# skywoodsz/qm_control

Hardware: NVIDIA H100
Metric: mpc_wbc_iters_per_s (higher is better)
Workload: dtype f64

## Files before the change

qm_control_b200/csrc/kernels/mpc_kernels.cu:

```cuda
#include <cstdlib>
#include "mpc_api.cuh"
#include "mpc_device.cuh"
#include "node_eval.cuh"
#include "wlinalg.cuh"

namespace qmb {

#ifndef QMB_LQ_WARPS
#define QMB_LQ_WARPS 4
#endif
#ifndef QMB_LQ_MINB
#define QMB_LQ_MINB 4
#endif
constexpr int LQ_WARPS = QMB_LQ_WARPS, LS_WARPS = 4, SETUP_WARPS = 4;
enum { MST_ITER_CAP = 1, MST_OVERFLOW = 2, MST_NAN = 4, MST_NOT_PD = 8, MST_NO_STEP = 16, MST_CONVERGED = 32, MST_NEG_DT = 64 };

__device__ __forceinline__ double interval_start(double t, int ev) { return ev == 2 ? t + WEAK_EPS : t; }
__device__ __forceinline__ double interval_end(double t, int ev) { return ev == 1 ? t - WEAK_EPS : t; }
__device__ __forceinline__ int clamp_events(int ne) { return ne < 0 ? 0 : (ne > EMAX ? EMAX : ne); }
__device__ __forceinline__ int clamp_targets(int nk) { return nk < 1 ? 1 : (nk > KMAX ? KMAX : nk); }
__device__ __forceinline__ int flag_mask(int mode) { int m = 0; for (int i = 0; i < 4; ++i) if (contact_flag(mode, i)) m |= 1 << i; return m; }

struct SetupIdx { int iu, ix; double au, ax; };
__host__ __device__ inline size_t setup_smem_per_warp(int nmax) { return (size_t)nmax * (8 + 8 + 4 + sizeof(SetupIdx) + 4) + 8 * EMAX + 64; }
// ... 59 lines not shown
  ne::NodeRec rec;
  QuadWs quad; LegWs leg[4];
  double x[NX], u[NU];
  double A1r[9 * NX], Ar[9 * NX];
  double Pe_full[NU], rs[NU];
  int dep_idx[MAXDEP], free_idx[MU], col_of_input[NU];
};
static_assert(9 * NX * 8 >= EMAX * 8 + EMAX + 8, "the mode schedule (event times + modes) is staged in the Ar buffer until the flow Jacobians are expanded");
static_assert(sizeof(LqLate) <= 4 * sizeof(ne::FootBlk) && offsetof(ne::NodeRec, foot) == 0, "LqLate overlays the foot blocks of the record");
static_assert(sizeof(LqSmem) % 16 == 0 && offsetof(LqSmem, rec) == 0, "aligned record slice");
static_assert((sizeof(LqSmem) * LQ_WARPS + 1024) * QMB_LQ_MINB <= 232448, "projection kernel: QMB_LQ_MINB CTAs of LQ_WARPS warps per SM (13.8 KB per node: four CTAs of four warps = 16 nodes in flight)");

#ifndef QMB_FL_MINB
#define QMB_FL_MINB 2
#endif
constexpr int FL_WARPS = 4, FL_TILE = 64;
constexpr int FL_SMEM = FL_WARPS * 32 * (FL_TILE + 1) * 8;
__global__ void __launch_bounds__(32 * FL_WARPS, QMB_FL_MINB) mpc_flow_kernel(const DevModel* __restrict__ mdl, int b0, int B, int nmax, MpcProblemDev p, MpcSolutionDev sol, double* __restrict__ rec, const int32_t* __restrict__ status) {
  extern __shared__ __align__(16) unsigned char smem_raw[]; double (*tile)[32][FL_TILE + 1] = reinterpret_cast<double (*)[32][FL_TILE + 1]>(smem_raw);
  const int tid = threadIdx.x, warp = tid >> 5, lane = tid & 31; const long long gid = (long long)blockIdx.x * (32 * FL_WARPS) + tid;
  const int b = b0 + (int)(gid / nmax), k = (int)(gid % nmax);
  const int n = (b < B) ? sol.n_nodes[b] : 0;
  bool work = b < B && k < n && !(status[b] & MST_CONVERGED);
  const bool terminal = work && (k == n - 1);
  if (work && !terminal && sol.event[(size_t)b * nmax + k] == 1) work = false;
  const unsigned active = __ballot_sync(FULL, work); if (!active) return;
  double* row = &tile[warp][lane][0]; double* gbase = rec + ((size_t)b0 * nmax + (size_t)(gid - lane)) * ne::NODE_REC_DBL;
  auto flush = [&](int off, int cnt) {
    __syncwarp();
#pragma unroll 4
    for (int rw = 0; rw < 32; ++rw) if ((active >> rw) & 1u) { double* g = gbase + (size_t)rw * ne::NODE_REC_DBL + off; if (lane < cnt) g[lane] = tile[warp][rw][lane]; if (lane + 32 < cnt) g[lane + 32] = tile[warp][rw][lane + 32]; }
    __syncwarp(); };
  double x[NX], u[NU]; ne::BaseKin bk; ne::FlowAcc acc; double t = 0.0, dt = 0.0;
  if (work) {
    const double* gt = sol.t + (size_t)b * nmax; const int32_t* ge = sol.event + (size_t)b * nmax;
    const double* xk = sol.x + ((size_t)b * nmax + k) * NX; const double* uk = sol.u + ((size_t)b * nmax + k) * NU;
#pragma unroll
    for (int i = 0; i < NX; ++i) { x[i] = xk[i]; u[i] = terminal ? 0.0 : uk[i]; }
    t = interval_start(gt[k], ge[k]); dt = terminal ? 0.0 : interval_end(gt[k + 1], ge[k + 1]) - t;
    ne::base_eval<true>(mdl, x, bk); ne::flow_acc_init(acc);
  }
#pragma unroll 1
  for (int i = 0; i < 4; ++i) {
    if (work) { ne::FootBlk* fb = reinterpret_cast<ne::FootBlk*>(row); double al[9];
      ne::foot_eval<true>(mdl, x, u, bk, i, acc, fb->d, fb->pf, fb->Jl, al, fb->JxF);
      if (!terminal) ne::foot_velocity_1<true>(mdl, x, u, bk, i, fb->d, fb->Jl, al, fb->e, fb->C); }
    flush(i * ne::FOOT_DBL, ne::FOOT_DBL);
  }
  double f1[12];
  if (work) { ne::FlowBlk* fl = reinterpret_cast<ne::FlowBlk*>(row); ne::flow_finish<true>(mdl, x, bk, acc, fl->f, fl);
#pragma unroll
    for (int i = 0; i < 12; ++i) f1[i] = fl->f[i]; }
  flush(4 * ne::FOOT_DBL, ne::FLOW_DBL);
  { ne::EeRec ee;
    if (work) { const int nk = clamp_targets(p.n_target[b]); const ne::TargetSeg sg = ne::target_segment(p.target_times + (size_t)b * KMAX, p.target_states + (size_t)b * KMAX * TARGET_DIM, nk, t);
      double pref[3], qref[4]; ne::target_pose(sg, nk, pref, qref); ne::ee_eval<true>(mdl, x, bk, pref, qref, ee.e, ee.Je);
#pragma unroll
      for (int j = 0; j < 39; ++j) row[j] = reinterpret_cast<const double*>(&ee)[j]; }
    flush(4 * ne::FOOT_DBL + ne::FLOW_DBL, 39);
    if (work) {
#pragma unroll
      for (int j = 0; j < 39; ++j) row[j] = reinterpret_cast<const double*>(&ee)[39 + j]; }
    flush(4 * ne::FOOT_DBL + ne::FLOW_DBL + 39, 39); }
  const bool stage2 = work && !terminal;
  if (stage2) {
    const double cdt = mdl->rk_c * dt;
#pragma unroll
    for (int i = 0; i < NX; ++i) x[i] += cdt * (i < 12 ? f1[i < 12 ? i : 0] : u[i]);
    ne::base_eval<true>(mdl, x, bk); ne::flow_acc_init(acc);
#pragma unroll 1
    for (int i = 0; i < 4; ++i) { ne::Foot2Blk* f2 = reinterpret_cast<ne::Foot2Blk*>(row) + i; ne::foot_eval<true>(mdl, x, u, bk, i, acc, f2->d, nullptr, nullptr, nullptr, f2->JxF); }
  }
  flush(4 * ne::FOOT_DBL + ne::FLOW_DBL + ne::EE_DBL, 4 * ne::FOOT2_DBL);
  if (stage2) { ne::FlowBlk* fl = reinterpret_cast<ne::FlowBlk*>(row); ne::flow_finish<true>(mdl, x, bk, acc, fl->f, fl); }
  flush(4 * ne::FOOT_DBL + ne::FLOW_DBL + ne::EE_DBL + 4 * ne::FOOT2_DBL, ne::FLOW_DBL);
}

__device__ __forceinline__ void expand_flow(const ne::FlowBlk& fb, const double* jxf0, int fstride , double* Ar, int lfp, int lane) {
// ... 544 lines not shown
  }
  armijo = warp_sum(armijo); dxn2 = warp_sum(dxn2); dun2 = warp_sum(dun2);
  __syncthreads();
  if (lane == 0) { sm.red[warp][0] = armijo; sm.red[warp][1] = dxn2; sm.red[warp][2] = dun2; }
  __syncthreads();
  if (tid == 0) { double a = 0, x2 = 0, u2 = 0; for (int w = 0; w < RIC_THREADS / 32; ++w) { a += sm.red[w][0]; x2 += sm.red[w][1]; u2 += sm.red[w][2]; }
    double* rb = robot + (size_t)b * ROBOT_DBL; rb[0] = a; rb[1] = perf[0]; rb[2] = perf[1]; rb[3] = perf[2]; rb[4] = sqrt(x2); rb[5] = sqrt(u2); if (st) atomicOr(&status[b], st); }
}

__device__ __forceinline__ void fixup_inputs(MpcSolutionDev sol, int b, int nmax, int n, int tid, int nthreads) {
  const int32_t* ge = sol.event + (size_t)b * nmax; double* gu = sol.u + (size_t)b * nmax * NU;
  for (int i = tid; i < NU; i += nthreads) for (int k = 1; k < n; ++k) if ((k == n - 1) || (ge[k] == 1)) gu[(size_t)k * NU + i] = gu[(size_t)(k - 1) * NU + i];
}

#ifndef QMB_LS_MINB
#define QMB_LS_MINB 4
#endif
__global__ void __launch_bounds__(32 * LS_WARPS, QMB_LS_MINB) mpc_linesearch_kernel(const DevModel* __restrict__ mdl, int b0, int B, int nmax, MpcProblemDev p, MpcSolutionDev sol, const double* __restrict__ dxo, const double* __restrict__ duo,
                                                                     const double* __restrict__ robot, int32_t* __restrict__ status, double* __restrict__ step_info, int iteration) {
  __shared__ double red[LS_WARPS][3]; __shared__ int decision; __shared__ double s_ev[EMAX]; __shared__ unsigned char s_modes[EMAX + 8];
  const int tid = threadIdx.x, warp = tid >> 5, lane = tid & 31; const int b = b0 + blockIdx.x; if (b >= B) return;
  if (status[b] & MST_CONVERGED) return;
  const int n = sol.n_nodes[b]; const int N = n - 1;
  const double* gt = sol.t + (size_t)b * nmax; const int32_t* ge = sol.event + (size_t)b * nmax;
  double* gx = sol.x + (size_t)b * nmax * NX; double* gu = sol.u + (size_t)b * nmax * NU; const double* gdx = dxo + (size_t)b * nmax * NX; const double* gdu = duo + (size_t)b * nmax * NU;
  const int ne = clamp_events(p.n_events[b]); const double* ev = s_ev; const unsigned char* modes = s_modes;
  if (tid < 32) { const double* gev = p.event_times + (size_t)b * EMAX; const int32_t* gmodes = p.modes + (size_t)b * (EMAX + 1); s_ev[lane] = (lane < ne) ? gev[lane] : 0.0; s_modes[lane] = (unsigned char)((lane <= ne) ? gmodes[lane] : 15); if (lane == 0) s_modes[EMAX] = (unsigned char)((EMAX <= ne) ? gmodes[EMAX] : 15); }
  __syncthreads();
  const int nk = clamp_targets(p.n_target[b]); const double* tt = p.target_times + (size_t)b * KMAX; const double* ts = p.target_states + (size_t)b * KMAX * TARGET_DIM;
  const double* rb = robot + (size_t)b * ROBOT_DBL; const double armijo = rb[0], base_cost = rb[1], base_viol = sqrt(rb[2] + rb[3]), dxn = rb[4], dun = rb[5];
  const bool failed = (status[b] & MST_NOT_PD) != 0;
  double alpha = 1.0; bool accepted = false; double sc = base_cost, sd = rb[2], se = rb[3];
  const double w1 = mdl->rk_w1, w2 = mdl->rk_w2;
  while (!failed) {
    double cost = 0.0, dyn = 0.0, eq = 0.0;
    for (int k = tid; k <= N; k += 32 * LS_WARPS) {
      double xa[NX], ua[NU]; const bool terminal = (k == N);
#pragma unroll
      for (int i = 0; i < NX; ++i) { xa[i] = gx[(size_t)k * NX + i] + alpha * gdx[(size_t)k * NX + i]; ua[i] = terminal ? 0.0 : gu[(size_t)k * NU + i] + alpha * gdu[(size_t)k * NU + i]; }
      if (k == 0) { double s = 0.0; for (int i = 0; i < NX; ++i) { const double d = p.x0[(size_t)b * NX + i] - xa[i]; s = fma(d, d, s); } dyn += s; }
      if (!terminal && ge[k] == 1) { double s = 0.0; for (int i = 0; i < NX; ++i) { const double d = xa[i] - (gx[(size_t)(k + 1) * NX + i] + alpha * gdx[(size_t)(k + 1) * NX + i]); s = fma(d, d, s); } dyn += s; continue; }
      const double t = interval_start(gt[k], ge[k]);
      const double dt = terminal ? 1.0 : interval_end(gt[k + 1], ge[k + 1]) - t; const int mode = mode_at_time(ev, modes, ne, t); const int fm = terminal ? 0 : flag_mask(mode);
      ne::BaseKin bk; ne::FlowAcc acc; double f1[12];
      ne::base_eval<false>(mdl, xa, bk); ne::flow_acc_init(acc);
      { double fe[4][3], pf[4][3];
#pragma unroll 1
        for (int i = 0; i < 4; ++i) { double d[3], Jl[9]; ne::foot_eval<false>(mdl, xa, ua, bk, i, acc, d, pf[i], Jl, nullptr, nullptr); if (!terminal) ne::foot_velocity_1<false>(mdl, xa, ua, bk, i, d, Jl, nullptr, fe[i], nullptr); }
        if (!terminal) eq += dt * ne::equality_ss(mdl, ua, fe, pf, fm, ev, modes, ne, t, nullptr); }
      ne::flow_finish<false>(mdl, xa, bk, acc, f1, nullptr);
      { const ne::TargetSeg sg = ne::target_segment(tt, ts, nk, t); double pref[3], qref[4], ee[6]; ne::target_pose(sg, nk, pref, qref); ne::ee_eval<false>(mdl, xa, bk, pref, qref, ee, nullptr);
        cost += dt * ne::cost_value(mdl, xa, ua, sg, ee, fm, terminal); }
      if (terminal) continue;
      const double cdt = mdl->rk_c * dt;
#pragma unroll
      for (int i = 0; i < NX; ++i) xa[i] += cdt * (i < 12 ? f1[i < 12 ? i : 0] : ua[i]);
      double f2[12]; ne::base_eval<false>(mdl, xa, bk); ne::flow_acc_init(acc);
#pragma unroll 1
      for (int i = 0; i < 4; ++i) { double d[3]; ne::foot_eval<false>(mdl, xa, ua, bk, i, acc, d, nullptr, nullptr, nullptr, nullptr); }
      ne::flow_finish<false>(mdl, xa, bk, acc, f2, nullptr);
      double s = 0.0;
#pragma unroll
      for (int i = 0; i < NX; ++i) { const double fa = (i < 12) ? f1[i < 12 ? i : 0] : ua[i], fb = (i < 12) ? f2[i < 12 ? i : 0] : ua[i];
        const double x0i = gx[(size_t)k * NX + i] + alpha * gdx[(size_t)k * NX + i];
        const double d = x0i + dt * (w1 * fa + w2 * fb) - (gx[(size_t)(k + 1) * NX + i] + alpha * gdx[(size_t)(k + 1) * NX + i]); s = fma(d, d, s); }
      dyn += dt * s;
    }
    cost = warp_sum(cost); dyn = warp_sum(dyn); eq = warp_sum(eq);
    if (lane == 0) { red[warp][0] = cost; red[warp][1] = dyn; red[warp][2] = eq; }
    __syncthreads();
    if (threadIdx.x == 0) {
      double c = 0, dd = 0, e = 0; for (int w = 0; w < LS_WARPS; ++w) { c += red[w][0]; dd += red[w][1]; e += red[w][2]; }
      const double sv = sqrt(dd + e), am = alpha * armijo; bool acc;
      if (sv > mdl->g_max) acc = sv < (1.0 - mdl->gamma_c) * base_viol;
      else if (sv < mdl->g_min && base_viol < mdl->g_min && am < 0.0) acc = c < base_cost + mdl->armijo_factor * am;
      else acc = (c < base_cost - mdl->gamma_c * base_viol) || (sv < (1.0 - mdl->gamma_c) * base_viol);
      red[0][0] = c; red[0][1] = dd; red[0][2] = e;
      int dec = 0; if (acc) dec = 1; else { const double an = alpha * mdl->alpha_decay; if ((an * dxn < mdl->delta_tol && an * dun < mdl->delta_tol) || an < mdl->alpha_min) dec = 2; }
      decision = dec;
    }
// ... 20 lines not shown
    int flags = accepted ? 0 : MST_NO_STEP;
    if (iteration + 1 < mdl->sqp_iterations) {
      const bool stepsize = alpha < mdl->alpha_min;
      const bool metrics = fabs(sc - base_cost) < mdl->cost_tol && sqrt(sd + se) < mdl->g_min;
      const bool primal = alpha * dxn < mdl->delta_tol && alpha * dun < mdl->delta_tol;
      if (stepsize || metrics || primal) flags |= MST_CONVERGED;
    }
    if (flags) atomicOr(&status[b], flags);
    double* si = step_info + (size_t)b * 4; si[0] = alpha; si[1] = sc; si[2] = sd; si[3] = se; }
}

constexpr int RO_THREADS = 128, RO_MAXTRIALS = 32;
template <bool PERF, class MT>
__device__ __forceinline__ void rollout_step(const DevModel* __restrict__ mdl, double* x, const double* u, double t, double dt, int fm, const double* ev, const MT* modes, int ne, const double* tt, const double* ts, int nk, double& cost, double& eq) {
  ne::BaseKin bk; ne::FlowAcc acc; double f1[12], x2[NX]; ne::base_eval<false>(mdl, x, bk); ne::flow_acc_init(acc);
  if (PERF) { double fe[4][3], pf[4][3];
#pragma unroll 1
    for (int i = 0; i < 4; ++i) { double d[3], Jl[9]; ne::foot_eval<false>(mdl, x, u, bk, i, acc, d, pf[i], Jl, nullptr, nullptr); ne::foot_velocity_1<false>(mdl, x, u, bk, i, d, Jl, nullptr, fe[i], nullptr); }
    eq += dt * ne::equality_ss(mdl, u, fe, pf, fm, ev, modes, ne, t, nullptr);
    const ne::TargetSeg sg = ne::target_segment(tt, ts, nk, t); double pref[3], qref[4], ee[6]; ne::target_pose(sg, nk, pref, qref); ne::ee_eval<false>(mdl, x, bk, pref, qref, ee, nullptr);
    cost += dt * ne::cost_value(mdl, x, u, sg, ee, fm, false);
  } else {
#pragma unroll 1
    for (int i = 0; i < 4; ++i) { double d[3]; ne::foot_eval<false>(mdl, x, u, bk, i, acc, d, nullptr, nullptr, nullptr, nullptr); } }
  ne::flow_finish<false>(mdl, x, bk, acc, f1, nullptr);
  const double cdt = mdl->rk_c * dt, w1 = mdl->rk_w1, w2 = mdl->rk_w2;
#pragma unroll
  for (int i = 0; i < NX; ++i) x2[i] = x[i] + cdt * (i < 12 ? f1[i < 12 ? i : 0] : u[i]);
  double f2[12]; ne::base_eval<false>(mdl, x2, bk); ne::flow_acc_init(acc);
#pragma unroll 1
  for (int i = 0; i < 4; ++i) { double d[3]; ne::foot_eval<false>(mdl, x2, u, bk, i, acc, d, nullptr, nullptr, nullptr, nullptr); }
  ne::flow_finish<false>(mdl, x2, bk, acc, f2, nullptr);
#pragma unroll
  for (int i = 0; i < NX; ++i) x[i] += dt * (w1 * (i < 12 ? f1[i < 12 ? i : 0] : u[i]) + w2 * (i < 12 ? f2[i < 12 ? i : 0] : u[i]));
// ... 138 lines not shown

bool mpc_alloc(MpcBuffers& m, int B, int nmax, std::string& err, std::vector<void*>& allocs, cudaStream_t stream) {
  m.B = B; m.nmax = nmax; m.cur = 0;
  if (SETUP_WARPS * ((setup_smem_per_warp(nmax) + 15) & ~(size_t)15) > 200 * 1024) { err = "max_nodes too large for the grid staging of the setup kernel (limit ~1000 nodes)"; return false; }
  auto A = [&](auto** p, size_t count) { void* q = nullptr; const size_t bytes = count * sizeof(**p); cudaError_t e = cudaMalloc(&q, bytes); if (e != cudaSuccess) { err = std::string("cudaMalloc (MPC buffers) failed: ") + cudaGetErrorString(e); return false; } cudaMemsetAsync(q, 0, bytes, stream); allocs.push_back(q); *p = static_cast<std::remove_reference_t<decltype(**p)>*>(q); return true; };
  const size_t Bn = (size_t)B * nmax;
  bool ok = A(&m.t0, B) && A(&m.x0, (size_t)B * NX) && A(&m.n_events, B) && A(&m.event_times, (size_t)B * EMAX) && A(&m.modes, (size_t)B * (EMAX + 1)) && A(&m.n_target, B) && A(&m.target_times, (size_t)B * KMAX) && A(&m.target_states, (size_t)B * KMAX * TARGET_DIM);
  for (int s = 0; s < 2 && ok; ++s) ok = A(&m.sol[s].n_nodes, B) && A(&m.sol[s].t, Bn) && A(&m.sol[s].event, Bn) && A(&m.sol[s].x, Bn * NX) && A(&m.sol[s].u, Bn * NU);
  ok = ok && A(&m.stage, Bn * STAGE_DBL) && A(&m.gains, Bn * GAIN_DBL) && A(&m.dx, Bn * NX) && A(&m.du, Bn * NU) && A(&m.node_rec, Bn * ne::NODE_REC_DBL) && A(&m.ddp_trial, (size_t)B * RO_MAXTRIALS * 2) && A(&m.robot, (size_t)B * ROBOT_DBL) && A(&m.status, B) && A(&m.step_info, (size_t)B * 4);
  return ok;
}

int mpc_configure_device() {
  cudaError_t e = cudaFuncSetAttribute(mpc_setup_kernel, cudaFuncAttributeMaxDynamicSharedMemorySize, 200 * 1024);
  if (e == cudaSuccess) e = cudaFuncSetAttribute(mpc_flow_kernel, cudaFuncAttributeMaxDynamicSharedMemorySize, FL_SMEM);
  if (e == cudaSuccess) e = cudaFuncSetAttribute(mpc_rollout_trials_kernel, cudaFuncAttributeMaxDynamicSharedMemorySize, RO_RPC_MAX * GAIN_DBL * 8);
  if (e == cudaSuccess) e = cudaFuncSetAttribute(mpc_lq_kernel, cudaFuncAttributeMaxDynamicSharedMemorySize, (int)(sizeof(LqSmem) * LQ_WARPS));
  if (e == cudaSuccess) e = cudaFuncSetAttribute(mpc_riccati_kernel, cudaFuncAttributeMaxDynamicSharedMemorySize, (int)sizeof(RicSmem));
  return (int)e;
}

int mpc_solve_launch(const DevModel* mdl, const DevModel& hm, MpcBuffers& m, const MpcProblemDev& p, int b0, int b1, cudaStream_t stream, cudaEvent_t* ev) {
  const int nb = b1 - b0, nmax = m.nmax; if (nb <= 0) return 0;
  MpcSolutionDev prev = m.sol[m.cur], next = m.sol[1 - m.cur];
  if (ev) cudaEventRecord(ev[0], stream);
  mpc_setup_kernel<<<(nb + SETUP_WARPS - 1) / SETUP_WARPS, 32 * SETUP_WARPS, SETUP_WARPS * ((setup_smem_per_warp(nmax) + 15) & ~(size_t)15), stream>>>(mdl, b0, b1, nmax, p, prev, next, m.status);
  if (ev) cudaEventRecord(ev[1], stream);
  const long long nodes = (long long)nb * nmax; const int iters = hm.sqp_iterations < 1 ? 1 : hm.sqp_iterations; int launched = 1;
  const bool ddp = hm.solver == 2; int n_trials = 0, tr_pitch = 1;
  if (ddp) { for (double a = hm.ddp_max_step; a >= hm.ddp_min_step && n_trials < RO_MAXTRIALS; a *= hm.ddp_contraction) ++n_trials; while (tr_pitch < n_trials) tr_pitch *= 2; }
  const int ro_grid = (nb + RO_THREADS - 1) / RO_THREADS; const int ro_rpc = (RO_THREADS / tr_pitch < RO_RPC_MAX) ? RO_THREADS / tr_pitch : RO_RPC_MAX;
  if (ddp) { mpc_rollout_kernel<<<ro_grid, RO_THREADS, 0, stream>>>(mdl, b0, b1, nmax, p, next, m.stage, m.gains, m.ddp_trial, m.robot, m.status, m.step_info, 0, 1, 1, 0); ++launched; }
  for (int it = 0; it < iters; ++it) {
    mpc_flow_kernel<<<(unsigned)((nodes + 32 * FL_WARPS - 1) / (32 * FL_WARPS)), 32 * FL_WARPS, FL_SMEM, stream>>>(mdl, b0, b1, nmax, p, next, m.node_rec, m.status);
    if (ev && it == iters - 1) cudaEventRecord(ev[7], stream);
    mpc_lq_kernel<<<(unsigned)((nodes + LQ_WARPS - 1) / LQ_WARPS), 32 * LQ_WARPS, sizeof(LqSmem) * LQ_WARPS, stream>>>(mdl, b0, b1, nmax, p, next, m.node_rec, m.stage, m.status);
    if (ev && it == iters - 1) cudaEventRecord(ev[2], stream);
    mpc_riccati_kernel<<<nb, RIC_THREADS, sizeof(RicSmem), stream>>>(mdl, b0, b1, nmax, p, next, m.stage, m.gains, m.dx, m.du, m.robot, m.status);
    if (ev && it == iters - 1) cudaEventRecord(ev[3], stream);
    if (ddp) { mpc_rollout_trials_kernel<<<(nb + ro_rpc - 1) / ro_rpc, ro_rpc * tr_pitch, (size_t)ro_rpc * GAIN_DBL * 8, stream>>>(mdl, b0, b1, nmax, p, next, m.stage, m.gains, m.ddp_trial, m.robot, m.status, n_trials, tr_pitch, ro_rpc);
      mpc_rollout_kernel<<<ro_grid, RO_THREADS, 0, stream>>>(mdl, b0, b1, nmax, p, next, m.stage, m.gains, m.ddp_trial, m.robot, m.status, m.step_info, 2, n_trials, tr_pitch, it); ++launched; }
    else mpc_linesearch_kernel<<<nb, 32 * LS_WARPS, 0, stream>>>(mdl, b0, b1, nmax, p, next, m.dx, m.du, m.robot, m.status, m.step_info, it);
    launched += 4;
  }
  if (ev) cudaEventRecord(ev[4], stream);
  return launched;
}

int mpc_policy_eval_launch(const MpcBuffers& m, const double* t, double* x_des, double* u_des, int32_t* mode, cudaStream_t stream, int b0, int b1) {
  if (b1 < 0) b1 = m.B; if (b1 <= b0) return 0;
  mpc_policy_eval_kernel<<<(b1 - b0 + 3) / 4, 128, 0, stream>>>(b0, b1, m.nmax, m.sol[m.cur], m.n_events, m.event_times, m.modes, t, x_des, u_des, mode);
  return 1;
}
int mpc_fixup_launch(const MpcBuffers& m, cudaStream_t stream) { mpc_fixup_kernel<<<m.B, 32, 0, stream>>>(m.B, m.nmax, m.sol[m.cur]); return 1; }

__global__ void __launch_bounds__(256) fp64_peak_kernel(double* out, int iters, double a, double b) {
  double x0 = threadIdx.x, x1 = x0 + 1, x2 = x0 + 2, x3 = x0 + 3, x4 = x0 + 4, x5 = x0 + 5, x6 = x0 + 6, x7 = x0 + 7;
// ... 17 lines not shown
```

qm_control_b200/csrc/kernels/node_eval.cuh:

```cuda
#pragma once
#include "mpc_scalar.cuh"

namespace qmb {
namespace ne {

struct FootBlk { double d[3], pf[3], Jl[9], JxF[9], e[3], C[3][12]; };
struct FlowBlk {
  double f[12];
  double Mpc[9], Mtw[9];
  double hth[3][3], vp[3][3], vt[3][3];
};
struct EeRec { double Je[6 * 12]; double e[6]; };
struct Foot2Blk { double d[3], JxF[9]; };
struct NodeRec { FootBlk foot[4]; FlowBlk s1; EeRec ee; Foot2Blk foot2[4]; FlowBlk s2; };
constexpr int FOOT_DBL = 63, FLOW_DBL = 57, EE_DBL = 78, FOOT2_DBL = 12;
constexpr int NODE_REC_DBL = 4 * FOOT_DBL + FLOW_DBL + EE_DBL + 4 * FOOT2_DBL + FLOW_DBL;
static_assert(sizeof(FootBlk) == FOOT_DBL * 8 && sizeof(FlowBlk) == FLOW_DBL * 8 && sizeof(EeRec) == EE_DBL * 8 && sizeof(Foot2Blk) == FOOT2_DBL * 8 && sizeof(NodeRec) == NODE_REC_DBL * 8, "the record is a flat array of doubles");
static_assert(sizeof(NodeRec) % 16 == 0, "records stay 16-byte aligned");

struct BaseKin { double tr[6], R0[9], T[9], Tinv[9], W[9], c[3], rcom[3], omega[3], thd[3], dom[3][3]; };
struct FlowAcc { double fsum[3], hang[3], hth[3][3]; };

template <int NJC>
QMB_HD void chain_fk(const DevModel* __restrict__ mdl, const double* R0, const double* p0, const double* qj, int first, double* Rl, double* pl, double (*org)[3], double (*axs)[3]) {
  double Rp[9], pp[3];
#pragma unroll
  for (int i = 0; i < 9; ++i) Rp[i] = R0[i];
  pp[0] = p0[0]; pp[1] = p0[1]; pp[2] = p0[2];
#pragma unroll
  for (int jj = 0; jj < NJC; ++jj) {
    const int j = first + jj; double s, c; sincos(qj[j], &s, &c);
    const int ax = mdl->axis[j]; const double* Rj = mdl->Rj[j]; double Rlq[9];
#pragma unroll
    for (int i = 0; i < 3; ++i) { const double r0 = Rj[3 * i], r1 = Rj[3 * i + 1], r2 = Rj[3 * i + 2];
      if (ax == 0) { Rlq[3 * i] = r0; Rlq[3 * i + 1] = c * r1 + s * r2; Rlq[3 * i + 2] = -s * r1 + c * r2; }
      else if (ax == 1) { Rlq[3 * i] = c * r0 - s * r2; Rlq[3 * i + 1] = r1; Rlq[3 * i + 2] = s * r0 + c * r2; }
      else { Rlq[3 * i] = c * r0 + s * r1; Rlq[3 * i + 1] = -s * r0 + c * r1; Rlq[3 * i + 2] = r2; } }
    double Rw[9], pw[3]; matmul3(Rp, Rlq, Rw); const double pj[3] = {mdl->pj[j][0], mdl->pj[j][1], mdl->pj[j][2]}; matvec3(Rp, pj, pw);
    pw[0] += pp[0]; pw[1] += pp[1]; pw[2] += pp[2];
    org[jj][0] = pw[0]; org[jj][1] = pw[1]; org[jj][2] = pw[2];
    axs[jj][0] = ax == 0 ? Rw[0] : (ax == 1 ? Rw[1] : Rw[2]); axs[jj][1] = ax == 0 ? Rw[3] : (ax == 1 ? Rw[4] : Rw[5]); axs[jj][2] = ax == 0 ? Rw[6] : (ax == 1 ? Rw[7] : Rw[8]);
#pragma unroll
    for (int i = 0; i < 9; ++i) Rp[i] = Rw[i];
    pp[0] = pw[0]; pp[1] = pw[1]; pp[2] = pw[2];
  }
#pragma unroll
// ... 13 lines not shown
#pragma unroll
      for (int bq = 0; bq < 3; ++bq) { const double rib = R[3 * i] * Ii[bq] + R[3 * i + 1] * Ii[3 + bq] + R[3 * i + 2] * Ii[6 + bq]; acc = fma(rib, R[3 * jj + bq], acc); }
      bk.W[3 * i + jj] = m * acc; }
  matvec3(R, mdl->c_nom, bk.c);
  for (int a = 0; a < 3; ++a) bk.rcom[a] = x[6 + a] - bk.c[a];
  matvec3(bk.W, ha, bk.omega); matvec3(bk.Tinv, bk.omega, bk.thd);
  if (JAC) { for (int k = 0; k < 3; ++k) { const double Tk[3] = {bk.T[k], bk.T[3 + k], bk.T[6 + k]}; double t1[3], t2[3], t3[3];
      cross3(Tk, bk.omega, t1); cross3(Tk, ha, t2); matvec3(bk.W, t2, t3); for (int a = 0; a < 3; ++a) bk.dom[k][a] = t1[a] - t3[a]; } }
}

QMB_HD void flow_acc_init(FlowAcc& acc) { for (int a = 0; a < 3; ++a) { acc.fsum[a] = 0.0; acc.hang[a] = 0.0; for (int k = 0; k < 3; ++k) acc.hth[k][a] = 0.0; } }

template <bool JAC>
QMB_HD void foot_eval(const DevModel* __restrict__ mdl, const double* x, const double* u, const BaseKin& bk, int i, FlowAcc& acc, double* d, double* pf, double* Jl, double* al, double* JxF) {
  const int first = mdl->foot_leg[i]; double Rl[9], pl[3], org[3][3], axs[3][3];
  chain_fk<3>(mdl, bk.R0, x + 6, x + 12, first, Rl, pl, org, axs);
  double pw[3]; matvec3(Rl, mdl->foot_p[i], pw);
  for (int a = 0; a < 3; ++a) { pw[a] += pl[a]; d[a] = pw[a] - bk.rcom[a]; if (pf) pf[a] = pw[a]; }
  const double* F = u + 3 * i; const double im = 1.0 / mdl->total_mass;
  for (int a = 0; a < 3; ++a) acc.fsum[a] += F[a];
  cross3_add(d, F, acc.hang);
  for (int j = 0; j < 3; ++j) { const double r[3] = {pw[0] - org[j][0], pw[1] - org[j][1], pw[2] - org[j][2]}; double col[3]; cross3(axs[j], r, col);
    if (Jl) for (int a = 0; a < 3; ++a) Jl[3 * j + a] = col[a];
    if (al) for (int a = 0; a < 3; ++a) al[3 * j + a] = axs[j][a];
    if (JAC) { double jf[3]; cross3(col, F, jf); for (int a = 0; a < 3; ++a) JxF[3 * j + a] = jf[a] * im; } }
  if (JAC) for (int k = 0; k < 3; ++k) { const double Tk[3] = {bk.T[k], bk.T[3 + k], bk.T[6 + k]}; double t[3]; cross3(Tk, d, t); cross3_add(t, F, acc.hth[k]); }
}

template <bool JAC>
QMB_HD void flow_finish(const DevModel* __restrict__ mdl, const double* x, const BaseKin& bk, const FlowAcc& acc, double* f, FlowBlk* fb) {
  const double im = 1.0 / mdl->total_mass; const double* om = bk.omega; const double* c = bk.c;
  for (int a = 0; a < 3; ++a) { f[a] = acc.fsum[a] * im + (a == 2 ? -9.81 : 0.0); f[3 + a] = acc.hang[a] * im; f[9 + a] = bk.thd[a]; }
  { double oc[3]; cross3(om, c, oc); for (int a = 0; a < 3; ++a) f[6 + a] = x[a] + oc[a]; }
  if (JAC) {
// ... 6 lines not shown
      const double Tk[3] = {bk.T[k], bk.T[3 + k], bk.T[6 + k]}; const double* domk = bk.dom[k];
      double tc[3], vpk[3]; cross3(Tk, c, tc); cross3(domk, c, vpk); cross3_add(om, tc, vpk);
      for (int a = 0; a < 3; ++a) { fb->vp[k][a] = vpk[a]; fb->hth[k][a] = acc.hth[k][a] * im; }
      const double tmp[3] = {domk[0] - dT[0], domk[1] - dT[1], domk[2] - dT[2]}; matvec3(bk.Tinv, tmp, fb->vt[k]);
    }
    const double* W = bk.W;
    for (int i = 0; i < 3; ++i) for (int jj = 0; jj < 3; ++jj) {
      const double s0 = (i == 0) ? 0.0 : (i == 1 ? c[2] : -c[1]), s1 = (i == 0) ? -c[2] : (i == 1 ? 0.0 : c[0]), s2 = (i == 0) ? c[1] : (i == 1 ? -c[0] : 0.0);
      fb->Mpc[3 * i + jj] = -(s0 * W[jj] + s1 * W[3 + jj] + s2 * W[6 + jj]);
      fb->Mtw[3 * i + jj] = bk.Tinv[3 * i] * W[jj] + bk.Tinv[3 * i + 1] * W[3 + jj] + bk.Tinv[3 * i + 2] * W[6 + jj]; }
  }
}

template <bool JAC>
QMB_HD void foot_velocity_1(const DevModel* __restrict__ mdl, const double* x, const double* u, const BaseKin& bk, int i, const double* d, const double* Jli, const double* ali, double* e, double (*C)[12]) {
  const int first = mdl->foot_leg[i]; const double* om = bk.omega; const double qd[3] = {u[12 + first], u[12 + first + 1], u[12 + first + 2]};
  double w[3] = {0, 0, 0}; for (int j = 0; j < 3; ++j) for (int a = 0; a < 3; ++a) w[a] += Jli[3 * j + a] * qd[j];
  double v[3]; cross3(om, d, v); for (int a = 0; a < 3; ++a) e[a] = v[a] + x[a] + w[a];
  if (JAC) {
    for (int a = 0; a < 3; ++a) for (int cc = 0; cc < 12; ++cc) C[a][cc] = (cc == a) ? 1.0 : 0.0;
    const double Sd[9] = {0, -d[2], d[1], d[2], 0, -d[0], -d[1], d[0], 0}; double SW[9]; matmul3(Sd, bk.W, SW);
    for (int a = 0; a < 3; ++a) for (int b = 0; b < 3; ++b) C[a][3 + b] = -SW[3 * a + b];
    for (int k = 0; k < 3; ++k) { const double Tk[3] = {bk.T[k], bk.T[3 + k], bk.T[6 + k]}; double t[3], col[3]; cross3(bk.dom[k], d, col); cross3(Tk, d, t); cross3_add(om, t, col); cross3_add(Tk, w, col); for (int a = 0; a < 3; ++a) C[a][6 + k] = col[a]; }
    for (int j = 0; j < 3; ++j) {
      const double* Jj = Jli + 3 * j; const double* aj = ali + 3 * j; double above[3] = {0, 0, 0}, below[3] = {0, 0, 0};
      for (int l = j + 1; l < 3; ++l) for (int a = 0; a < 3; ++a) above[a] += Jli[3 * l + a] * qd[l];
      for (int l = 0; l <= j; ++l) for (int a = 0; a < 3; ++a) below[a] += ali[3 * l + a] * qd[l];
      double col[3]; cross3(om, Jj, col); cross3_add(aj, above, col); cross3_add(below, Jj, col);
      for (int a = 0; a < 3; ++a) C[a][9 + j] = col[a];
    }
  }
// ... 6 lines not shown
QMB_HD void target_pose(const TargetSeg& sg, int nk, double* pref, double* qref) {
  const double* l = sg.l; const double* rr = sg.rr; const double a = sg.a;
  for (int i = 0; i < 3; ++i) pref[i] = a * l[30 + i] + (1.0 - a) * rr[30 + i];
  if (nk > 1) {
    const double* ql = l + 33; const double* qr = rr + 33; const double tq = 1.0 - a; double d = 0.0; for (int i = 0; i < 4; ++i) d += ql[i] * qr[i];
    const double ad = fabs(d); double s0, s1;
    if (ad >= 1.0 - 2.220446049250313e-16) { s0 = 1.0 - tq; s1 = tq; } else { const double th = acos(ad), st = sin(th); const double ist = 1.0 / st; s0 = sin((1.0 - tq) * th) * ist; s1 = sin(tq * th) * ist; }
    if (d < 0.0) s1 = -s1;
    for (int i = 0; i < 4; ++i) qref[i] = s0 * ql[i] + s1 * qr[i];
  } else { for (int i = 0; i < 4; ++i) qref[i] = l[33 + i]; }
}

template <bool JAC>
QMB_HD void ee_eval(const DevModel* __restrict__ mdl, const double* x, const BaseKin& bk, const double* pref, const double* qref, double* e, double* Je ) {
  double Rl[9], pl[3], org[6][3], axs[6][3];
  chain_fk<6>(mdl, bk.R0, x + 6, x + 12, 12, Rl, pl, org, axs);
  double R[9]; matmul3(Rl, mdl->ee_R, R); double pw[3]; matvec3(Rl, mdl->ee_p, pw);
  for (int a = 0; a < 3; ++a) { pw[a] += pl[a]; e[a] = pw[a] - pref[a]; }
  double q[4]; const double tr = R[0] + R[4] + R[8];
  if (tr > 0.0) { const double s = sqrt(tr + 1.0) * 2.0, is = 1.0 / s; q[0] = 0.25 * s; q[1] = (R[7] - R[5]) * is; q[2] = (R[2] - R[6]) * is; q[3] = (R[3] - R[1]) * is; }
  else if (R[0] > R[4] && R[0] > R[8]) { const double s = sqrt(1.0 + R[0] - R[4] - R[8]) * 2.0, is = 1.0 / s; q[0] = (R[7] - R[5]) * is; q[1] = 0.25 * s; q[2] = (R[1] + R[3]) * is; q[3] = (R[2] + R[6]) * is; }
  else if (R[4] > R[8]) { const double s = sqrt(1.0 + R[4] - R[0] - R[8]) * 2.0, is = 1.0 / s; q[0] = (R[2] - R[6]) * is; q[1] = (R[1] + R[3]) * is; q[2] = 0.25 * s; q[3] = (R[5] + R[7]) * is; }
  else { const double s = sqrt(1.0 + R[8] - R[0] - R[4]) * 2.0, is = 1.0 / s; q[0] = (R[3] - R[1]) * is; q[1] = (R[2] + R[6]) * is; q[2] = (R[5] + R[7]) * is; q[3] = 0.25 * s; }
  const double* rv = qref; const double rw = qref[3]; const double* qv = q + 1; double cr[3]; cross3(qv, rv, cr);
  for (int a = 0; a < 3; ++a) e[3 + a] = q[0] * rv[a] - rw * qv[a] + cr[a];
  if (JAC) {
    for (int cidx = 0; cidx < 12; ++cidx) {
      double n[3] = {0, 0, 0}, lin[3] = {0, 0, 0};
      if (cidx < 3) lin[cidx] = 1.0;
      else if (cidx < 6) { const int k = cidx - 3; n[0] = bk.T[k]; n[1] = bk.T[3 + k]; n[2] = bk.T[6 + k]; const double r[3] = {pw[0] - x[6], pw[1] - x[7], pw[2] - x[8]}; cross3(n, r, lin); }
      else { const int j = cidx - 6; n[0] = axs[j][0]; n[1] = axs[j][1]; n[2] = axs[j][2]; const double r[3] = {pw[0] - org[j][0], pw[1] - org[j][1], pw[2] - org[j][2]}; cross3(n, r, lin); }
      const double dw = -0.5 * dot3(n, qv); double dv[3]; cross3(n, qv, dv); for (int a = 0; a < 3; ++a) dv[a] = 0.5 * (q[0] * n[a] + dv[a]);
      double cr2[3]; cross3(dv, rv, cr2);
      for (int a = 0; a < 3; ++a) { Je[a * 12 + cidx] = lin[a]; Je[(3 + a) * 12 + cidx] = dw * rv[a] - rw * dv[a] + cr2[a]; }
    }
  }
}

QMB_HD double cost_value(const DevModel* __restrict__ mdl, const double* x, const double* u, const TargetSeg& sg, const double* ee, int flagmask, bool terminal) {
  double value = 0.0;
  if (!terminal) {
    int nst = 0; for (int i = 0; i < 4; ++i) nst += (flagmask >> i) & 1;
    double dx[NX], du[NU];
    for (int i = 0; i < NX; ++i) { dx[i] = x[i] - (sg.a * sg.l[i] + (1.0 - sg.a) * sg.rr[i]); double un = 0.0; if (i < 12 && (i % 3) == 2 && ((flagmask >> (i / 3)) & 1)) un = mdl->total_mass * 9.81 / nst; du[i] = u[i] - un; }
    double acc = 0.0;
    if (mdl->q_is_diag) { for (int i = 0; i < NX; ++i) acc = fma(dx[i] * mdl->Qdiag[i], dx[i], acc); }
    else { for (int i = 0; i < NX; ++i) { double qd = 0.0; for (int j = 0; j < NX; ++j) qd = fma(mdl->Q[i * NX + j], dx[j], qd); acc = fma(dx[i], qd, acc); } }
    for (int blk = 0; blk < 8; ++blk) { const double* Rb = mdl->Rblk[blk]; const double* d3 = du + 3 * blk;
      for (int r = 0; r < 3; ++r) acc = fma(d3[r], fma(Rb[3 * r], d3[0], fma(Rb[3 * r + 1], d3[1], Rb[3 * r + 2] * d3[2])), acc); }
    for (int i = 0; i < 6; ++i) acc = fma(du[24 + i] * mdl->Rarm[i], du[24 + i], acc);
    value += 0.5 * acc;
  }
  { const double mup = terminal ? mdl->mu_final_ee_pos : mdl->mu_ee_pos, muo = terminal ? mdl->mu_final_ee_ori : mdl->mu_ee_ori;
    double v = 0.0; for (int r = 0; r < 6; ++r) v += 0.5 * (r < 3 ? mup : muo) * ee[r] * ee[r]; value += v; }
  if (!terminal) {
    double bv = 0.0;
    for (int grp = 0; grp < 2; ++grp) {
      const bool pos = grp == 0; const double mu = pos ? mdl->pos_limit_mu : mdl->vel_limit_mu, de = pos ? mdl->pos_limit_delta : mdl->vel_limit_delta; double prod = 1.0;
      for (int i = 0; i < 6; ++i) { const double val = pos ? x[24 + i] : u[24 + i]; const double lo = pos ? mdl->arm_pos_lower[i] : mdl->arm_vel_lower[i], hi = pos ? mdl->arm_pos_upper[i] : mdl->arm_vel_upper[i];
        const double h2[2] = {val - lo, hi - val};
        for (int sd = 0; sd < 2; ++sd) { const double h = h2[sd]; if (h > de) prod *= h; else { const double tq = (h - 2.0 * de) / de; bv += mu * (-log(de) + 0.5 * tq * tq - 0.5); } } }
      bv -= mu * log(prod); }
    { double prod = 1.0; const double mu = mdl->friction_barrier_mu, de = mdl->friction_barrier_delta;
      for (int i = 0; i < 4; ++i) if ((flagmask >> i) & 1) { const double Fx = u[3 * i], Fy = u[3 * i + 1], Fz = u[3 * i + 2]; const double h = mdl->friction_mu * Fz - sqrt(Fx * Fx + Fy * Fy + mdl->friction_reg);
        if (h > de) prod *= h; else { const double tq = (h - 2.0 * de) / de; bv += mu * (-log(de) + 0.5 * tq * tq - 0.5); } }
      bv -= mu * log(prod); }
    value += bv;
  }
  return value;
}

template <class MT>
QMB_HD double equality_ss(const DevModel* __restrict__ mdl, const double* u, const double (*e)[3], const double (*pf)[3], int flagmask, const double* ev, const MT* modes, int ne, double t, bool* swing_ok) {
  double es = 0.0; bool ok = true;
  for (int i = 0; i < 4; ++i) {
    if ((flagmask >> i) & 1) { for (int a = 0; a < 3; ++a) es += e[i][a] * e[i][a]; }
    else { double zp, zv; ok &= swing_reference(mdl, ev, modes, ne, i, t, zp, zv); double ez = e[i][2] - zv; if (mdl->position_error_gain != 0.0) ez += mdl->position_error_gain * (pf[i][2] - zp);
      es += ez * ez; for (int a = 0; a < 3; ++a) es += u[3 * i + a] * u[3 * i + a]; }
  }
  if (swing_ok) *swing_ok = ok;
  return es;
}

}
}
```

Baseline: 19.42.

## Cut register pressure in flow and line-search kernels by staging state in shared memory

The flow kernel now keeps the control vector u in a per-thread shared-memory row and writes the end-effector record straight into the staging tile in a single flush. The line-search kernel stages its trial state, control and first flow in dynamic shared memory, and its occupancy hint drops from four blocks to two. Foot and cost helpers use pick3 selects instead of dynamically indexed local arrays, and the equality term is accumulated per foot, so fewer per-thread arrays spill to local memory. The cost is more shared-memory traffic and a larger shared footprint, which may lower the number of resident blocks.

```diff
diff --git a/qm_control_b200/csrc/kernels/mpc_kernels.cu b/qm_control_b200/csrc/kernels/mpc_kernels.cu
--- a/qm_control_b200/csrc/kernels/mpc_kernels.cu
+++ b/qm_control_b200/csrc/kernels/mpc_kernels.cu
@@ -97,8 +97,9 @@
 #ifndef QMB_FL_MINB
 #define QMB_FL_MINB 2
 #endif
-constexpr int FL_WARPS = 4, FL_TILE = 64;
-constexpr int FL_SMEM = FL_WARPS * 32 * (FL_TILE + 1) * 8;
+constexpr int FL_WARPS = 4, FL_TILE = ne::EE_DBL;
+constexpr int FL_UROW = NU + 1;
+constexpr int FL_SMEM = FL_WARPS * 32 * (FL_TILE + 1 + FL_UROW) * 8;
 __global__ void __launch_bounds__(32 * FL_WARPS, QMB_FL_MINB) mpc_flow_kernel(const DevModel* __restrict__ mdl, int b0, int B, int nmax, MpcProblemDev p, MpcSolutionDev sol, double* __restrict__ rec, const int32_t* __restrict__ status) {
   extern __shared__ __align__(16) unsigned char smem_raw[]; double (*tile)[32][FL_TILE + 1] = reinterpret_cast<double (*)[32][FL_TILE + 1]>(smem_raw);
   const int tid = threadIdx.x, warp = tid >> 5, lane = tid & 31; const long long gid = (long long)blockIdx.x * (32 * FL_WARPS) + tid;
@@ -112,14 +113,18 @@
   auto flush = [&](int off, int cnt) {
     __syncwarp();
 #pragma unroll 4
-    for (int rw = 0; rw < 32; ++rw) if ((active >> rw) & 1u) { double* g = gbase + (size_t)rw * ne::NODE_REC_DBL + off; if (lane < cnt) g[lane] = tile[warp][rw][lane]; if (lane + 32 < cnt) g[lane + 32] = tile[warp][rw][lane + 32]; }
+    for (int rw = 0; rw < 32; ++rw) if ((active >> rw) & 1u) { double* g = gbase + (size_t)rw * ne::NODE_REC_DBL + off;
+#pragma unroll
+      for (int c = lane; c < FL_TILE; c += 32) if (c < cnt) g[c] = tile[warp][rw][c]; }
     __syncwarp(); };
-  double x[NX], u[NU]; ne::BaseKin bk; ne::FlowAcc acc; double t = 0.0, dt = 0.0;
+  double* u = reinterpret_cast<double*>(smem_raw + (size_t)FL_WARPS * 32 * (FL_TILE + 1) * 8) + tid * FL_UROW;
+  double x[NX]; ne::BaseKin bk; ne::FlowAcc acc; double t = 0.0, dt = 0.0;
   if (work) {
     const double* gt = sol.t + (size_t)b * nmax; const int32_t* ge = sol.event + (size_t)b * nmax;
     const double* xk = sol.x + ((size_t)b * nmax + k) * NX; const double* uk = sol.u + ((size_t)b * nmax + k) * NU;
 #pragma unroll
     for (int i = 0; i < NX; ++i) { x[i] = xk[i]; u[i] = terminal ? 0.0 : uk[i]; }
+    asm volatile("" ::: "memory");
     t = interval_start(gt[k], ge[k]); dt = terminal ? 0.0 : interval_end(gt[k + 1], ge[k + 1]) - t;
     ne::base_eval<true>(mdl, x, bk); ne::flow_acc_init(acc);
   }
@@ -135,16 +140,10 @@
 #pragma unroll
     for (int i = 0; i < 12; ++i) f1[i] = fl->f[i]; }
   flush(4 * ne::FOOT_DBL, ne::FLOW_DBL);
-  { ne::EeRec ee;
-    if (work) { const int nk = clamp_targets(p.n_target[b]); const ne::TargetSeg sg = ne::target_segment(p.target_times + (size_t)b * KMAX, p.target_states + (size_t)b * KMAX * TARGET_DIM, nk, t);
-      double pref[3], qref[4]; ne::target_pose(sg, nk, pref, qref); ne::ee_eval<true>(mdl, x, bk, pref, qref, ee.e, ee.Je);
-#pragma unroll
-      for (int j = 0; j < 39; ++j) row[j] = reinterpret_cast<const double*>(&ee)[j]; }
-    flush(4 * ne::FOOT_DBL + ne::FLOW_DBL, 39);
-    if (work) {
-#pragma unroll
-      for (int j = 0; j < 39; ++j) row[j] = reinterpret_cast<const double*>(&ee)[39 + j]; }
-    flush(4 * ne::FOOT_DBL + ne::FLOW_DBL + 39, 39); }
+  if (work) { ne::EeRec* ee = reinterpret_cast<ne::EeRec*>(row);
+    const int nk = clamp_targets(p.n_target[b]); const ne::TargetSeg sg = ne::target_segment(p.target_times + (size_t)b * KMAX, p.target_states + (size_t)b * KMAX * TARGET_DIM, nk, t);
+    double pref[3], qref[4]; ne::target_pose(sg, nk, pref, qref); ne::ee_eval<true>(mdl, x, bk, pref, qref, ee->e, ee->Je); }
+  flush(4 * ne::FOOT_DBL + ne::FLOW_DBL, ne::EE_DBL);
   const bool stage2 = work && !terminal;
   if (stage2) {
     const double cdt = mdl->rk_c * dt;
@@ -719,11 +718,13 @@
 }
 
 #ifndef QMB_LS_MINB
-#define QMB_LS_MINB 4
+#define QMB_LS_MINB 2
 #endif
+constexpr int LS_ROW = NX + NU + 12 + 1, LS_SMEM = 32 * LS_WARPS * LS_ROW * 8;
 __global__ void __launch_bounds__(32 * LS_WARPS, QMB_LS_MINB) mpc_linesearch_kernel(const DevModel* __restrict__ mdl, int b0, int B, int nmax, MpcProblemDev p, MpcSolutionDev sol, const double* __restrict__ dxo, const double* __restrict__ duo,
                                                                      const double* __restrict__ robot, int32_t* __restrict__ status, double* __restrict__ step_info, int iteration) {
   __shared__ double red[LS_WARPS][3]; __shared__ int decision; __shared__ double s_ev[EMAX]; __shared__ unsigned char s_modes[EMAX + 8];
+  extern __shared__ double s_tp[];
   const int tid = threadIdx.x, warp = tid >> 5, lane = tid & 31; const int b = b0 + blockIdx.x; if (b >= B) return;
   if (status[b] & MST_CONVERGED) return;
   const int n = sol.n_nodes[b]; const int N = n - 1;
@@ -740,35 +741,42 @@
   while (!failed) {
     double cost = 0.0, dyn = 0.0, eq = 0.0;
     for (int k = tid; k <= N; k += 32 * LS_WARPS) {
-      double xa[NX], ua[NU]; const bool terminal = (k == N);
-#pragma unroll
+      double* xa = s_tp + tid * LS_ROW; double* ua = xa + NX; const bool terminal = (k == N);
+#pragma unroll 6
       for (int i = 0; i < NX; ++i) { xa[i] = gx[(size_t)k * NX + i] + alpha * gdx[(size_t)k * NX + i]; ua[i] = terminal ? 0.0 : gu[(size_t)k * NU + i] + alpha * gdu[(size_t)k * NU + i]; }
+      asm volatile("" ::: "memory");
       if (k == 0) { double s = 0.0; for (int i = 0; i < NX; ++i) { const double d = p.x0[(size_t)b * NX + i] - xa[i]; s = fma(d, d, s); } dyn += s; }
       if (!terminal && ge[k] == 1) { double s = 0.0; for (int i = 0; i < NX; ++i) { const double d = xa[i] - (gx[(size_t)(k + 1) * NX + i] + alpha * gdx[(size_t)(k + 1) * NX + i]); s = fma(d, d, s); } dyn += s; continue; }
       const double t = interval_start(gt[k], ge[k]);
       const double dt = terminal ? 1.0 : interval_end(gt[k + 1], ge[k + 1]) - t; const int mode = mode_at_time(ev, modes, ne, t); const int fm = terminal ? 0 : flag_mask(mode);
-      ne::BaseKin bk; ne::FlowAcc acc; double f1[12];
+      ne::BaseKin bk; ne::FlowAcc acc; double* f1 = ua + NU;
       ne::base_eval<false>(mdl, xa, bk); ne::flow_acc_init(acc);
-      { double fe[4][3], pf[4][3];
+      { double es = 0.0; bool ok = true;
 #pragma unroll 1
-        for (int i = 0; i < 4; ++i) { double d[3], Jl[9]; ne::foot_eval<false>(mdl, xa, ua, bk, i, acc, d, pf[i], Jl, nullptr, nullptr); if (!terminal) ne::foot_velocity_1<false>(mdl, xa, ua, bk, i, d, Jl, nullptr, fe[i], nullptr); }
-        if (!terminal) eq += dt * ne::equality_ss(mdl, ua, fe, pf, fm, ev, modes, ne, t, nullptr); }
+        for (int i = 0; i < 4; ++i) { double d[3], Jl[9], pf[3]; ne::foot_eval<false>(mdl, xa, ua, bk, i, acc, d, pf, Jl, nullptr, nullptr);
+          if (!terminal) { double fe[3]; ne::foot_velocity_1<false>(mdl, xa, ua, bk, i, d, Jl, nullptr, fe, nullptr); ne::equality_add(mdl, ua, fe, pf, fm, ev, modes, ne, t, i, es, ok); } }
+        if (!terminal) eq += dt * es; }
       ne::flow_finish<false>(mdl, xa, bk, acc, f1, nullptr);
+      asm volatile("" ::: "memory");
       { const ne::TargetSeg sg = ne::target_segment(tt, ts, nk, t); double pref[3], qref[4], ee[6]; ne::target_pose(sg, nk, pref, qref); ne::ee_eval<false>(mdl, xa, bk, pref, qref, ee, nullptr);
         cost += dt * ne::cost_value(mdl, xa, ua, sg, ee, fm, terminal); }
       if (terminal) continue;
       const double cdt = mdl->rk_c * dt;
 #pragma unroll
-      for (int i = 0; i < NX; ++i) xa[i] += cdt * (i < 12 ? f1[i < 12 ? i : 0] : ua[i]);
+      for (int i = 0; i < 12; ++i) xa[i] += cdt * f1[i];
+#pragma unroll 6
+      for (int i = 12; i < NX; ++i) xa[i] += cdt * ua[i];
       double f2[12]; ne::base_eval<false>(mdl, xa, bk); ne::flow_acc_init(acc);
 #pragma unroll 1
       for (int i = 0; i < 4; ++i) { double d[3]; ne::foot_eval<false>(mdl, xa, ua, bk, i, acc, d, nullptr, nullptr, nullptr, nullptr); }
       ne::flow_finish<false>(mdl, xa, bk, acc, f2, nullptr);
       double s = 0.0;
-#pragma unroll
-      for (int i = 0; i < NX; ++i) { const double fa = (i < 12) ? f1[i < 12 ? i : 0] : ua[i], fb = (i < 12) ? f2[i < 12 ? i : 0] : ua[i];
-        const double x0i = gx[(size_t)k * NX + i] + alpha * gdx[(size_t)k * NX + i];
-        const double d = x0i + dt * (w1 * fa + w2 * fb) - (gx[(size_t)(k + 1) * NX + i] + alpha * gdx[(size_t)(k + 1) * NX + i]); s = fma(d, d, s); }
+      auto defect = [&](int i, double fa, double fb) { const double x0i = gx[(size_t)k * NX + i] + alpha * gdx[(size_t)k * NX + i];
+        const double d = x0i + dt * (w1 * fa + w2 * fb) - (gx[(size_t)(k + 1) * NX + i] + alpha * gdx[(size_t)(k + 1) * NX + i]); s = fma(d, d, s); };
+#pragma unroll
+      for (int i = 0; i < 12; ++i) defect(i, f1[i], f2[i]);
+#pragma unroll 6
+      for (int i = 12; i < NX; ++i) defect(i, ua[i], ua[i]);
       dyn += dt * s;
     }
     cost = warp_sum(cost); dyn = warp_sum(dyn); eq = warp_sum(eq);
@@ -819,10 +827,11 @@
 template <bool PERF, class MT>
 __device__ __forceinline__ void rollout_step(const DevModel* __restrict__ mdl, double* x, const double* u, double t, double dt, int fm, const double* ev, const MT* modes, int ne, const double* tt, const double* ts, int nk, double& cost, double& eq) {
   ne::BaseKin bk; ne::FlowAcc acc; double f1[12], x2[NX]; ne::base_eval<false>(mdl, x, bk); ne::flow_acc_init(acc);
-  if (PERF) { double fe[4][3], pf[4][3];
+  if (PERF) { double es = 0.0; bool ok = true;
 #pragma unroll 1
-    for (int i = 0; i < 4; ++i) { double d[3], Jl[9]; ne::foot_eval<false>(mdl, x, u, bk, i, acc, d, pf[i], Jl, nullptr, nullptr); ne::foot_velocity_1<false>(mdl, x, u, bk, i, d, Jl, nullptr, fe[i], nullptr); }
-    eq += dt * ne::equality_ss(mdl, u, fe, pf, fm, ev, modes, ne, t, nullptr);
+    for (int i = 0; i < 4; ++i) { double d[3], Jl[9], pf[3], fe[3]; ne::foot_eval<false>(mdl, x, u, bk, i, acc, d, pf, Jl, nullptr, nullptr); ne::foot_velocity_1<false>(mdl, x, u, bk, i, d, Jl, nullptr, fe, nullptr);
+      ne::equality_add(mdl, u, fe, pf, fm, ev, modes, ne, t, i, es, ok); }
+    eq += dt * es;
     const ne::TargetSeg sg = ne::target_segment(tt, ts, nk, t); double pref[3], qref[4], ee[6]; ne::target_pose(sg, nk, pref, qref); ne::ee_eval<false>(mdl, x, bk, pref, qref, ee, nullptr);
     cost += dt * ne::cost_value(mdl, x, u, sg, ee, fm, false);
   } else {
@@ -991,6 +1000,7 @@
 int mpc_configure_device() {
   cudaError_t e = cudaFuncSetAttribute(mpc_setup_kernel, cudaFuncAttributeMaxDynamicSharedMemorySize, 200 * 1024);
   if (e == cudaSuccess) e = cudaFuncSetAttribute(mpc_flow_kernel, cudaFuncAttributeMaxDynamicSharedMemorySize, FL_SMEM);
+  if (e == cudaSuccess) e = cudaFuncSetAttribute(mpc_linesearch_kernel, cudaFuncAttributeMaxDynamicSharedMemorySize, LS_SMEM);
   if (e == cudaSuccess) e = cudaFuncSetAttribute(mpc_rollout_trials_kernel, cudaFuncAttributeMaxDynamicSharedMemorySize, RO_RPC_MAX * GAIN_DBL * 8);
   if (e == cudaSuccess) e = cudaFuncSetAttribute(mpc_lq_kernel, cudaFuncAttributeMaxDynamicSharedMemorySize, (int)(sizeof(LqSmem) * LQ_WARPS));
   if (e == cudaSuccess) e = cudaFuncSetAttribute(mpc_riccati_kernel, cudaFuncAttributeMaxDynamicSharedMemorySize, (int)sizeof(RicSmem));
@@ -1017,7 +1027,7 @@
     if (ev && it == iters - 1) cudaEventRecord(ev[3], stream);
     if (ddp) { mpc_rollout_trials_kernel<<<(nb + ro_rpc - 1) / ro_rpc, ro_rpc * tr_pitch, (size_t)ro_rpc * GAIN_DBL * 8, stream>>>(mdl, b0, b1, nmax, p, next, m.stage, m.gains, m.ddp_trial, m.robot, m.status, n_trials, tr_pitch, ro_rpc);
       mpc_rollout_kernel<<<ro_grid, RO_THREADS, 0, stream>>>(mdl, b0, b1, nmax, p, next, m.stage, m.gains, m.ddp_trial, m.robot, m.status, m.step_info, 2, n_trials, tr_pitch, it); ++launched; }
-    else mpc_linesearch_kernel<<<nb, 32 * LS_WARPS, 0, stream>>>(mdl, b0, b1, nmax, p, next, m.dx, m.du, m.robot, m.status, m.step_info, it);
+    else mpc_linesearch_kernel<<<nb, 32 * LS_WARPS, LS_SMEM, stream>>>(mdl, b0, b1, nmax, p, next, m.dx, m.du, m.robot, m.status, m.step_info, it);
     launched += 4;
   }
   if (ev) cudaEventRecord(ev[4], stream);
diff --git a/qm_control_b200/csrc/kernels/node_eval.cuh b/qm_control_b200/csrc/kernels/node_eval.cuh
--- a/qm_control_b200/csrc/kernels/node_eval.cuh
+++ b/qm_control_b200/csrc/kernels/node_eval.cuh
@@ -21,15 +21,17 @@
 struct BaseKin { double tr[6], R0[9], T[9], Tinv[9], W[9], c[3], rcom[3], omega[3], thd[3], dom[3][3]; };
 struct FlowAcc { double fsum[3], hang[3], hth[3][3]; };
 
+QMB_HD double pick3(const double* a, int s, int c) { return s == 0 ? a[c] : (s == 1 ? a[3 + c] : (s == 2 ? a[6 + c] : a[9 + c])); }
+
 template <int NJC>
-QMB_HD void chain_fk(const DevModel* __restrict__ mdl, const double* R0, const double* p0, const double* qj, int first, double* Rl, double* pl, double (*org)[3], double (*axs)[3]) {
+QMB_HD void chain_fk(const DevModel* __restrict__ mdl, const double* R0, const double* p0, const double* q, int first, double* Rl, double* pl, double (*org)[3], double (*axs)[3]) {
   double Rp[9], pp[3];
 #pragma unroll
   for (int i = 0; i < 9; ++i) Rp[i] = R0[i];
   pp[0] = p0[0]; pp[1] = p0[1]; pp[2] = p0[2];
 #pragma unroll
   for (int jj = 0; jj < NJC; ++jj) {
-    const int j = first + jj; double s, c; sincos(qj[j], &s, &c);
+    const int j = first + jj; double s, c; sincos(q[jj], &s, &c);
     const int ax = mdl->axis[j]; const double* Rj = mdl->Rj[j]; double Rlq[9];
 #pragma unroll
     for (int i = 0; i < 3; ++i) { const double r0 = Rj[3 * i], r1 = Rj[3 * i + 1], r2 = Rj[3 * i + 2];
@@ -73,10 +75,11 @@
 template <bool JAC>
 QMB_HD void foot_eval(const DevModel* __restrict__ mdl, const double* x, const double* u, const BaseKin& bk, int i, FlowAcc& acc, double* d, double* pf, double* Jl, double* al, double* JxF) {
   const int first = mdl->foot_leg[i]; double Rl[9], pl[3], org[3][3], axs[3][3];
-  chain_fk<3>(mdl, bk.R0, x + 6, x + 12, first, Rl, pl, org, axs);
+  const double q[3] = {pick3(x + 12, first / 3, 0), pick3(x + 12, first / 3, 1), pick3(x + 12, first / 3, 2)};
+  chain_fk<3>(mdl, bk.R0, x + 6, q, first, Rl, pl, org, axs);
   double pw[3]; matvec3(Rl, mdl->foot_p[i], pw);
   for (int a = 0; a < 3; ++a) { pw[a] += pl[a]; d[a] = pw[a] - bk.rcom[a]; if (pf) pf[a] = pw[a]; }
-  const double* F = u + 3 * i; const double im = 1.0 / mdl->total_mass;
+  const double F[3] = {pick3(u, i, 0), pick3(u, i, 1), pick3(u, i, 2)}; const double im = 1.0 / mdl->total_mass;
   for (int a = 0; a < 3; ++a) acc.fsum[a] += F[a];
   cross3_add(d, F, acc.hang);
   for (int j = 0; j < 3; ++j) { const double r[3] = {pw[0] - org[j][0], pw[1] - org[j][1], pw[2] - org[j][2]}; double col[3]; cross3(axs[j], r, col);
@@ -113,7 +116,7 @@
 
 template <bool JAC>
 QMB_HD void foot_velocity_1(const DevModel* __restrict__ mdl, const double* x, const double* u, const BaseKin& bk, int i, const double* d, const double* Jli, const double* ali, double* e, double (*C)[12]) {
-  const int first = mdl->foot_leg[i]; const double* om = bk.omega; const double qd[3] = {u[12 + first], u[12 + first + 1], u[12 + first + 2]};
+  const int leg = mdl->foot_leg[i] / 3; const double* om = bk.omega; const double qd[3] = {pick3(u + 12, leg, 0), pick3(u + 12, leg, 1), pick3(u + 12, leg, 2)};
   double w[3] = {0, 0, 0}; for (int j = 0; j < 3; ++j) for (int a = 0; a < 3; ++a) w[a] += Jli[3 * j + a] * qd[j];
   double v[3]; cross3(om, d, v); for (int a = 0; a < 3; ++a) e[a] = v[a] + x[a] + w[a];
   if (JAC) {
@@ -150,7 +153,7 @@
 template <bool JAC>
 QMB_HD void ee_eval(const DevModel* __restrict__ mdl, const double* x, const BaseKin& bk, const double* pref, const double* qref, double* e, double* Je ) {
   double Rl[9], pl[3], org[6][3], axs[6][3];
-  chain_fk<6>(mdl, bk.R0, x + 6, x + 12, 12, Rl, pl, org, axs);
+  chain_fk<6>(mdl, bk.R0, x + 6, x + 24, 12, Rl, pl, org, axs);
   double R[9]; matmul3(Rl, mdl->ee_R, R); double pw[3]; matvec3(Rl, mdl->ee_p, pw);
   for (int a = 0; a < 3; ++a) { pw[a] += pl[a]; e[a] = pw[a] - pref[a]; }
   double q[4]; const double tr = R[0] + R[4] + R[8];
@@ -177,14 +180,16 @@
   double value = 0.0;
   if (!terminal) {
     int nst = 0; for (int i = 0; i < 4; ++i) nst += (flagmask >> i) & 1;
-    double dx[NX], du[NU];
-    for (int i = 0; i < NX; ++i) { dx[i] = x[i] - (sg.a * sg.l[i] + (1.0 - sg.a) * sg.rr[i]); double un = 0.0; if (i < 12 && (i % 3) == 2 && ((flagmask >> (i / 3)) & 1)) un = mdl->total_mass * 9.81 / nst; du[i] = u[i] - un; }
+    auto dx = [&](int i) { return x[i] - (sg.a * sg.l[i] + (1.0 - sg.a) * sg.rr[i]); };
+    const double un = mdl->total_mass * 9.81 / nst;
     double acc = 0.0;
-    if (mdl->q_is_diag) { for (int i = 0; i < NX; ++i) acc = fma(dx[i] * mdl->Qdiag[i], dx[i], acc); }
-    else { for (int i = 0; i < NX; ++i) { double qd = 0.0; for (int j = 0; j < NX; ++j) qd = fma(mdl->Q[i * NX + j], dx[j], qd); acc = fma(dx[i], qd, acc); } }
-    for (int blk = 0; blk < 8; ++blk) { const double* Rb = mdl->Rblk[blk]; const double* d3 = du + 3 * blk;
+    if (mdl->q_is_diag) { for (int i = 0; i < NX; ++i) { const double d = dx(i); acc = fma(d * mdl->Qdiag[i], d, acc); } }
+    else { for (int i = 0; i < NX; ++i) { double qd = 0.0; for (int j = 0; j < NX; ++j) qd = fma(mdl->Q[i * NX + j], dx(j), qd); acc = fma(dx(i), qd, acc); } }
+#pragma unroll
+    for (int blk = 0; blk < 8; ++blk) { const double* Rb = mdl->Rblk[blk];
+      const double d3[3] = {u[3 * blk], u[3 * blk + 1], u[3 * blk + 2] - ((blk < 4 && ((flagmask >> blk) & 1)) ? un : 0.0)};
       for (int r = 0; r < 3; ++r) acc = fma(d3[r], fma(Rb[3 * r], d3[0], fma(Rb[3 * r + 1], d3[1], Rb[3 * r + 2] * d3[2])), acc); }
-    for (int i = 0; i < 6; ++i) acc = fma(du[24 + i] * mdl->Rarm[i], du[24 + i], acc);
+    for (int i = 0; i < 6; ++i) acc = fma(u[24 + i] * mdl->Rarm[i], u[24 + i], acc);
     value += 0.5 * acc;
   }
   { const double mup = terminal ? mdl->mu_final_ee_pos : mdl->mu_ee_pos, muo = terminal ? mdl->mu_final_ee_ori : mdl->mu_ee_ori;
@@ -207,13 +212,15 @@
 }
 
 template <class MT>
+QMB_HD void equality_add(const DevModel* __restrict__ mdl, const double* u, const double* e, const double* pf, int flagmask, const double* ev, const MT* modes, int ne, double t, int i, double& es, bool& ok) {
+  if ((flagmask >> i) & 1) { for (int a = 0; a < 3; ++a) es += e[a] * e[a]; }
+  else { double zp, zv; ok &= swing_reference(mdl, ev, modes, ne, i, t, zp, zv); double ez = e[2] - zv; if (mdl->position_error_gain != 0.0) ez += mdl->position_error_gain * (pf[2] - zp);
+    es += ez * ez; for (int a = 0; a < 3; ++a) { const double F = pick3(u, i, a); es += F * F; } }
+}
+template <class MT>
 QMB_HD double equality_ss(const DevModel* __restrict__ mdl, const double* u, const double (*e)[3], const double (*pf)[3], int flagmask, const double* ev, const MT* modes, int ne, double t, bool* swing_ok) {
   double es = 0.0; bool ok = true;
-  for (int i = 0; i < 4; ++i) {
-    if ((flagmask >> i) & 1) { for (int a = 0; a < 3; ++a) es += e[i][a] * e[i][a]; }
-    else { double zp, zv; ok &= swing_reference(mdl, ev, modes, ne, i, t, zp, zv); double ez = e[i][2] - zv; if (mdl->position_error_gain != 0.0) ez += mdl->position_error_gain * (pf[i][2] - zp);
-      es += ez * ez; for (int a = 0; a < 3; ++a) es += u[3 * i + a] * u[3 * i + a]; }
-  }
+  for (int i = 0; i < 4; ++i) equality_add(mdl, u, e[i], pf[i], flagmask, ev, modes, ne, t, i, es, ok);
   if (swing_ok) *swing_ok = ok;
   return es;
 }
```

After: 20.33 (median of 6 runs). 1.05x the previous value.
